# AIoT-MLSys-Lab/Mercury

Measured on AMD Instinct MI355X. Metric: images/sec (whole node) + sampler overhead %, ResNet-18 CIFAR-10 DP 1/2/4/8 GPU, higher is better.
Workload: dtype bf16; 1 GPU; model=resnet18, dataset=cifar10-shape (32x32x3, 10 classes), global_batch=32, per_gpu_batch=32, presample_pool=320, optimizer=adam, parallelism=dp1, sampler=importance (loss + 0.5*EMA), with replacement

## Files before the change

csrc/igemm.h:

```cpp
#pragma once
#include <hip/hip_runtime.h>
#include <stddef.h>

typedef __bf16 bf16;

struct ConvGeom {
  int SH, SW, SC;
  int RP, RQ;
  int R, S, stride, pad;
  int Kc;
  int Ncols;
  int M;
  const bf16* zero;
  int ldb = 0;
  int trb = -1, tsb = 0, tS = 0;
};

constexpr int SUMS_R = 8;

struct EpiParams {
  bf16* out;
  int ldo;
  const float* bias;
  float* stats;
  int stats_ld;
  int group_rows;
  int accumulate;
  float* slab;
  const bf16* bw_out;
  const bf16* bw_y;
  const float* bw_stats;
  const bf16* bw_y2;
  const float* bw_stats2;
  float* bw_sums;
  float bw_inv_count, bw_eps;
  int bw_act;
  int rm_hc = 0, rm_wc = 0, rm_h = 0, rm_w = 0, rm_ph = 0, rm_pw = 0;
};

struct ProParams {
  const float* stats;
  const float* rmean;
  const float* rvar;
  const float* gamma;
  const float* beta;
  bf16* keep;
  int group_rows;
  float inv_count;
  float eps;
  int act;
  int keep_tap;
  const bf16* res = nullptr;
};

size_t igemm_slab_bytes(const ConvGeom& g, int bm, int bn, int splits);
void igemm_launch(const bf16* src, const bf16* wt, const ConvGeom& g, const EpiParams& e, int bm,
                  int bn, int splits, bool trans, hipStream_t st, const ProParams* pro = nullptr);

struct WgradGeom {
  int N, H, W, C;
  int P, Q, K;
  int R, S, stride, pad;
  int Creal;
  const bf16* zero;
  float* slab;
};
void wgrad_launch(const bf16* dy, const bf16* x, const WgradGeom& g, float* dw, int bm, int bn,
                  int splits, hipStream_t st);

int dgrad_s2_launch(const bf16* dy, const bf16* wt, const ConvGeom& g, const EpiParams& e, int bm,
                    int bn, int H, int W, int N, hipStream_t st);

int conv_bwd_pair_s2_launch(const bf16* dy, const bf16* wt, const ConvGeom& g, const EpiParams& e,
                            int bm, int bn, int H, int W, int N, const bf16* x,
                            const WgradGeom& wg, float* dw, int wbm, int wbn, int wsplits,
                            hipStream_t st);

int conv_bwd_pair_launch(const bf16* dy, const bf16* wt, const ConvGeom& g, const EpiParams& e,
                         int bm, int bn, int splits, const bf16* x, const WgradGeom& wg, float* dw,
                         int wbm, int wbn, int wsplits, hipStream_t st);

struct HconvGeom {
  int N, H, W, C;
  int P, Q, K;
  int R, stride, pad;
  int IMG, TR;
  int HT, HWd;
  int HWP, HALF;
  int HS, SR;
  int HPIX;
  int SWA;
  int PGRID;
  int chunks_per_split;
  const bf16* zero;
};

struct HconvPro {
  int mode;
  const float* stats;
  const float* rmean;
  const float* rvar;
  const float* gamma;
  const float* beta;
  int group_imgs;
  float inv_count;
  float eps;
  int act;
  int coef_tab = 0;
};

struct PgemmArgs {
  const bf16* a;
  const bf16* b;
  bf16* out;
  float* stats;
  int M, N, K, ldo, stats_ld, group_rows;
  unsigned a_bytes, b_bytes, out_bytes;
  int H, W, P, Q, stride;
};
struct PgemmPro {
  int mode;
  const float* stats;
  const float* rmean;
  const float* rvar;
  const float* gamma;
  const float* beta;
  float inv_count, eps;
  int act;
  int group_rows;
  int G;
  float* coef;
  const bf16* res;
  bf16* keep;
  unsigned res_bytes, keep_bytes, coef_bytes;
};
int pgemm_launch(const PgemmArgs& g, int bn, int grid, hipStream_t st, const PgemmPro* pro = nullptr);
int pwconv_launch(const PgemmArgs& g, hipStream_t st, const PgemmPro* pro = nullptr);

int hconv_launch(const bf16* src, const bf16* wt, const HconvGeom& g, const EpiParams& e,
                 const HconvPro& pro, int bm, int bn, int splits, hipStream_t st);
const bf16* conv_zero_page();
```

csrc/igemm.hip:

```cpp

#include "conv_epi.h"
#include "wgrad_body.h"

namespace {


__device__ __attribute__((aligned(16))) bf16 g_zero_page[64];

MA_DEV int swz(int row, int chunk) { return chunk ^ (row & 7); }

template <int BM, int BN>
constexpr int nt_occ() { return BM * BN >= 256 * 128 ? 1 : 2; }


template <bool TRANS>
MA_DEV void row_init(const ConvGeom& g, int m, int& off, int& h, int& w) {
  const int pq = g.RP * g.RQ;
  const int mm = m < g.M ? m : 0;
  const int n = udiv24(mm, pq, 1.f / (float)pq), rem = mm - n * pq;
  const int p = udiv24(rem, g.RQ, 1.f / (float)g.RQ), q = rem - p * g.RQ;
  off = m < g.M ? n * g.SH * g.SW : -1;
  h = TRANS ? p + g.pad : p * g.stride - g.pad;
  w = TRANS ? q + g.pad : q * g.stride - g.pad;
}

template <bool TRANS>
MA_DEV int row_at(const ConvGeom& g, int off, int h, int w, int r, int s, int c8) {
  int hh, ww;
  bool ok = off >= 0;
  if (TRANS) {
    const int hp = h - r, wp = w - s;
    if (g.stride == 2) {
      ok = ok && ((hp | wp) & 1) == 0;
      hh = hp >> 1;
      ww = wp >> 1;
    } else {
      hh = hp;
      ww = wp;
    }
  } else {
    hh = h + r;
    ww = w + s;
  }
  ok = ok && (unsigned)hh < (unsigned)g.SH && (unsigned)ww < (unsigned)g.SW;
  const int o = (off + hh * g.SW + ww) * g.SC + c8 * 8;
  return ok ? o : -1;
}

template <bool TRANS>
MA_DEV int row_base(const ConvGeom& g, int off, int h, int w) {
  if (TRANS && g.stride == 2) return (off + (h >> 1) * g.SW + (w >> 1)) * g.SC;
  return (off + h * g.SW + w) * g.SC;
}

template <bool TRANS>
MA_DEV int tap_offset(const ConvGeom& g, int r, int s) {
  if (!TRANS) return (r * g.SW + s) * g.SC;
  if (g.stride == 2) return -((r >> 1) * g.SW + (s >> 1)) * g.SC;
  return -(r * g.SW + s) * g.SC;
}

template <bool TRANS>
MA_DEV bool tap_ok(const ConvGeom& g, int h, int w, int r, int s) {
  if (!TRANS) return (unsigned)(h + r) < (unsigned)g.SH && (unsigned)(w + s) < (unsigned)g.SW;
  const int hp = h - r, wp = w - s;
  if (g.stride == 2)
    return ((hp | wp) & 1) == 0 && (unsigned)(hp >> 1) < (unsigned)g.SH &&
           (unsigned)(wp >> 1) < (unsigned)g.SW;
  return (unsigned)hp < (unsigned)g.SH && (unsigned)wp < (unsigned)g.SW;
}

struct KCursor {
  int tr, ts, tc;
  bool fast;
  MA_DEV void init(const ConvGeom& g, int kt0) {
    const int C8 = g.SC >> 3;
    fast = (C8 & 7) == 0;
    tr = ts = tc = 0;
    if (fast) {
      const int k0c = kt0 * 8;
      const int rs = k0c / C8;
      tc = k0c - rs * C8;
      tr = rs / g.S;
      ts = rs - tr * g.S;
    }
  }
  MA_DEV void decode(const ConvGeom& g, int kt, int lcc, int& r, int& s, int& c8, bool& kval) const {
    const int kc = kt * 8 + lcc;
    kval = kc < g.Kc;
    if (fast) {
      r = tr;
      s = ts;
      c8 = tc + lcc;
    } else {
      const int C8 = g.SC >> 3;
      const int k0 = kt * 8;
      int rs = k0 / C8;
      c8 = k0 - rs * C8 + lcc;
      while (c8 >= C8) {
        c8 -= C8;
        ++rs;
      }
      r = (int)(((float)rs + 0.5f) * (1.f / (float)g.S));
      s = rs - r * g.S;
    }
  }
  MA_DEV void advance(const ConvGeom& g) {
    if (!fast) return;
    tc += 8;
    if (tc == (g.SC >> 3)) {
      tc = 0;
      if (++ts == g.S) {
        ts = 0;
        ++tr;
      }
    }
  }
};

template <int BM, int BN>
MA_DEV void mma_stage(const bf16* a, const bf16* b, f32x4 (&acc)[BM / 32][BN / 32], int lane,
                      int wm, int wn) {
  constexpr int TM = BM / 32, TN = BN / 32;
#pragma unroll
  for (int kk = 0; kk < 2; ++kk) {
    const int chunk = kk * 4 + (lane >> 4);
    bf16x8 fa[TM], fb[TN];
#pragma unroll
    for (int tm = 0; tm < TM; ++tm) {
      const int row = wm * (BM / 2) + tm * 16 + (lane & 15);
      fa[tm] = *(const bf16x8*)(a + row * BK + swz(row, chunk) * 8);
    }
#pragma unroll
    for (int tn = 0; tn < TN; ++tn) {
      const int row = wn * (BN / 2) + tn * 16 + (lane & 15);
      fb[tn] = *(const bf16x8*)(b + row * BK + swz(row, chunk) * 8);
    }
#pragma unroll
    for (int tm = 0; tm < TM; ++tm)
#pragma unroll
      for (int tn = 0; tn < TN; ++tn)
        acc[tm][tn] = __builtin_amdgcn_mfma_f32_16x16x32_bf16(fb[tn], fa[tm], acc[tm][tn], 0, 0, 0);
  }
}

template <int BM, int BN, bool TRANS, bool PRO = false, int PF = 1>
MA_DEV void igemm_nt_body(const bf16* __restrict__ src, const bf16* __restrict__ wt,
                          const ConvGeom& g, const EpiParams& e, int ktiles_per_split, char* smem,
                          int bx, int by, int gx, int gy, const ProParams& pro) {
  constexpr int TM = BM / 32, TN = BN / 32;
  constexpr int AR = BM / 32, BR = BN / 32;
  bf16* sA = (bf16*)smem;

  const int tid = threadIdx.x, lane = tid & 63, w = tid >> 6;
  const int wm = w >> 1, wn = w & 1;
  const int ntn = (g.Ncols + BN - 1) / BN;
  const int mt = bx / ntn, nt = bx - mt * ntn;
  const int m0 = mt * BM, n0 = nt * BN;
  MA_STAMP(0);
  const int ktiles = (g.Kc + 7) / 8;
  const int kt0 = by * ktiles_per_split;
  const int kt1 = min(ktiles, kt0 + ktiles_per_split);
  const int Kelems = g.Kc * 8;
  const int cc = tid & 7;

  int abase[AR], ah[AR], aw[AR];
#pragma unroll
  for (int i = 0; i < AR; ++i) {
    int off;
    row_init<TRANS>(g, m0 + (tid >> 3) + 32 * i, off, ah[i], aw[i]);
    abase[i] = row_base<TRANS>(g, off, ah[i], aw[i]);
    if (off < 0) ah[i] = -(1 << 28);
  }
  int boff[BR];
  const int ldb = g.ldb ? g.ldb : Kelems;
#pragma unroll
  for (int i = 0; i < BR; ++i) {
    const int n = n0 + (tid >> 3) + 32 * i;
    boff[i] = n < g.Ncols ? n * ldb : -1;
  }
  KCursor kc;
  kc.init(g, kt0);
  const bf16* zp = g.zero;

  float4 pst[8];
  int pz = 0;
  int pko[AR];
  u32x4 prs[AR];
  const float* pbase = nullptr;
  if constexpr (PRO) {
    const int grp = m0 / pro.group_rows;
    pbase = pro.stats ? pro.stats + (size_t)grp * 2 * g.SC : nullptr;
  }
  auto load_stage = [&](int kt, u32x4 (&ra)[AR], u32x4 (&rb)[BR]) {
    int r, s, c8;
    bool kval;
    kc.decode(g, kt, cc, r, s, c8, kval);
    kc.advance(g);
    kval = kval && kt < kt1;
    bool keep = false;
    if constexpr (PRO) {
      const int ch = kval ? c8 * 8 : 0;
      const float* m0p = pbase ? pbase + ch : pro.rmean + ch;
      const float* v0p = pbase ? pbase + g.SC + ch : pro.rvar + ch;
      pst[0] = *(const float4*)m0p;
      pst[1] = *(const float4*)(m0p + 4);
      pst[2] = *(const float4*)v0p;
      pst[3] = *(const float4*)(v0p + 4);
      pst[4] = *(const float4*)(pro.gamma + ch);
      pst[5] = *(const float4*)(pro.gamma + ch + 4);
      pst[6] = *(const float4*)(pro.beta + ch);
      pst[7] = *(const float4*)(pro.beta + ch + 4);
      keep = pro.keep != nullptr && nt == 0 && kval && r * g.S + s == pro.keep_tap;
      pz = 0;
    }
    const int toff = tap_offset<TRANS>(g, r, s) + c8 * 8;
    const int bch = g.trb < 0 ? kt * 8 + cc
                              : ((g.trb - 2 * r) * g.tS + (g.tsb - 2 * s)) * (g.SC >> 3) + c8;
#pragma unroll
    for (int i = 0; i < AR; ++i) {
      const bool ok = kval && tap_ok<TRANS>(g, ah[i], aw[i], r, s);
      const int o = abase[i] + toff;
      ra[i] = *(const u32x4*)(ok ? src + o : zp);
      if constexpr (PRO) {
        pz |= (ok ? 0 : 1) << i;
        pko[i] = keep && ok ? o : -1;
        if (pro.res != nullptr) prs[i] = *(const u32x4*)(ok ? pro.res + o : zp);
      }
    }
#pragma unroll
    for (int i = 0; i < BR; ++i) {
      const bool ok = kval && boff[i] >= 0;
      rb[i] = *(const u32x4*)(ok ? wt + boff[i] + bch * 8 : zp);
    }
  };
  auto store_stage = [&](int buf, u32x4 (&ra)[AR], const u32x4 (&rb)[BR]) {
    bf16* a = sA + buf * Smem<BM, BN>::STAGE;
    bf16* b = a + BM * BK;
    if constexpr (PRO) {
      const float mv[8] = {pst[0].x, pst[0].y, pst[0].z, pst[0].w, pst[1].x, pst[1].y, pst[1].z, pst[1].w};
      const float vv[8] = {pst[2].x, pst[2].y, pst[2].z, pst[2].w, pst[3].x, pst[3].y, pst[3].z, pst[3].w};
      const float gv[8] = {pst[4].x, pst[4].y, pst[4].z, pst[4].w, pst[5].x, pst[5].y, pst[5].z, pst[5].w};
      const float bv[8] = {pst[6].x, pst[6].y, pst[6].z, pst[6].w, pst[7].x, pst[7].y, pst[7].z, pst[7].w};
      float sc[8], sh[8];
      float plo, phi;
      act_clamp_bounds(pro.act, plo, phi);
#pragma unroll
      for (int k = 0; k < 8; ++k) {
        float mean = mv[k], var = vv[k];
        if (pbase) {
          mean = mv[k] * pro.inv_count;
          var = fmaxf(vv[k] * pro.inv_count - mean * mean, 0.f);
        }
        sc[k] = gv[k] * rsqrtf(var + pro.eps);
        sh[k] = bv[k] - mean * sc[k];
      }
      const bool hres = pro.res != nullptr;
#pragma unroll
      for (int i = 0; i < AR; ++i) {
        const bf16x8 y = __builtin_bit_cast(bf16x8, ra[i]);
        const bf16x8 rv = __builtin_bit_cast(bf16x8, hres ? prs[i] : u32x4{0u, 0u, 0u, 0u});
        bf16x8 o;
#pragma unroll
        for (int k = 0; k < 8; ++k) {
          o[k] = f2bf(fminf(fmaxf(bf2f(y[k]) * sc[k] + sh[k] + bf2f(rv[k]), plo), phi));
        }
        const u32x4 t = __builtin_bit_cast(u32x4, o);
        ra[i] = ((pz >> i) & 1) ? u32x4{0u, 0u, 0u, 0u} : t;
        if (pko[i] >= 0) *(u32x4*)(pro.keep + pko[i]) = ra[i];
      }
    }
#pragma unroll
    for (int i = 0; i < AR; ++i) {
      const int row = (tid >> 3) + 32 * i;
      *(u32x4*)(a + row * BK + swz(row, cc) * 8) = ra[i];
    }
#pragma unroll
    for (int i = 0; i < BR; ++i) {
      const int row = (tid >> 3) + 32 * i;
      *(u32x4*)(b + row * BK + swz(row, cc) * 8) = rb[i];
    }
  };

  f32x4 acc[TM][TN];
#pragma unroll
  for (int i = 0; i < TM; ++i)
#pragma unroll
    for (int j = 0; j < TN; ++j) acc[i][j] = f32x4{0.f, 0.f, 0.f, 0.f};

  if (kt0 < kt1 && PF == 2) {
    u32x4 ra0[AR], rb0[BR], ra1[AR], rb1[BR];
    load_stage(kt0, ra0, rb0);
    store_stage(0, ra0, rb0);
    load_stage(kt0 + 1, ra1, rb1);
    __syncthreads();
    for (int kt = kt0; kt < kt1; kt += 2) {
      load_stage(kt + 2, ra0, rb0);
      mma_stage<BM, BN>(sA, sA + BM * BK, acc, lane, wm, wn);
      if (kt + 1 >= kt1) break;
      store_stage(1, ra1, rb1);
      __syncthreads();
      load_stage(kt + 3, ra1, rb1);
      const bf16* a1 = sA + Smem<BM, BN>::STAGE;
      mma_stage<BM, BN>(a1, a1 + BM * BK, acc, lane, wm, wn);
      if (kt + 2 >= kt1) break;
      store_stage(0, ra0, rb0);
      __syncthreads();
    }
    __syncthreads();
  } else if (kt0 < kt1) {
    u32x4 ra[AR], rb[BR];
    load_stage(kt0, ra, rb);
    store_stage(0, ra, rb);
    __syncthreads();
    MA_STAMP(1);
#ifdef MERCURY_STAMPS
    unsigned long long lap[4] = {0, 0, 0, 0};
    unsigned long long tl = __builtin_amdgcn_s_memtime();
#endif
    int buf = 0;
    for (int kt = kt0; kt < kt1; ++kt) {
      const bool more = kt + 1 < kt1;
      if (more) load_stage(kt + 1, ra, rb);
      MA_LAP(0, tl);
      const bf16* a = sA + buf * Smem<BM, BN>::STAGE;
      mma_stage<BM, BN>(a, a + BM * BK, acc, lane, wm, wn);
      MA_LAP(1, tl);
      if (more) store_stage(buf ^ 1, ra, rb);
      MA_LAP(2, tl);
      __syncthreads();
      MA_LAP(3, tl);
      buf ^= 1;
    }
#ifdef MERCURY_STAMPS
    if (threadIdx.x == 0) {
      const int b_ = blockIdx.x + blockIdx.y * gridDim.x;
      if (b_ < 8192)
        for (int q = 0; q < 4; ++q) g_stamps[b_][4 + q] = lap[q];
    }
#endif
  }
  MA_STAMP(2);
  finish<BM, BN>(acc, smem, e, g.M, g.Ncols, m0, n0, bx, by, gx, gy);
  MA_STAMP(3);
}


template <int BM, int BN>
constexpr int PAIR_PF() { return BM * BN <= 64 * 128 ? 2 : 1; }

template <int BM, int BN, bool TRANS, int PF = 1>
__global__ __launch_bounds__(NT, (nt_occ<BM, BN>())) void igemm_nt_kernel(const bf16* __restrict__ src,
                                                          const bf16* __restrict__ wt,
                                                          ConvGeom g, EpiParams e,
                                                          int ktiles_per_split) {
  __shared__ __attribute__((aligned(16))) char smem[Smem<BM, BN>::bytes(2)];
  const ProParams none{};
  const int bx = gridDim.y == 1 ? xcd_tile(blockIdx.x, gridDim.x) : blockIdx.x;
  igemm_nt_body<BM, BN, TRANS, false, PF>(src, wt, g, e, ktiles_per_split, smem, bx, blockIdx.y,
                                          gridDim.x, gridDim.y, none);
}

template <int BM, int BN>
__global__ __launch_bounds__(NT, (nt_occ<BM, BN>())) void igemm_pro_kernel(const bf16* __restrict__ src,
                                                           const bf16* __restrict__ wt,
                                                           ConvGeom g, EpiParams e,
                                                           int ktiles_per_split, ProParams pro) {
  __shared__ __attribute__((aligned(16))) char smem[Smem<BM, BN>::bytes(2)];
  const int bx = gridDim.y == 1 ? xcd_tile(blockIdx.x, gridDim.x) : blockIdx.x;
  igemm_nt_body<BM, BN, false, true>(src, wt, g, e, ktiles_per_split, smem, bx,
                                     blockIdx.y, gridDim.x, gridDim.y, pro);
}

template <int BM, int BN, bool TRANS>
void launch_main(const bf16* src, const bf16* wt, const ConvGeom& g, const EpiParams& e, int per,
                 dim3 grid, hipStream_t st) {
  if constexpr (PAIR_PF<BM, BN>() == 2) {
#ifndef MERCURY_FWD_PF1
    if (grid.x * grid.y <= 512) {
      hipLaunchKernelGGL((igemm_nt_kernel<BM, BN, TRANS, 2>), grid, dim3(NT), 0, st, src, wt, g, e,
                         per);
      return;
    }
#endif
  }
  hipLaunchKernelGGL((igemm_nt_kernel<BM, BN, TRANS>), grid, dim3(NT), 0, st, src, wt, g, e, per);
}

inline void ig_grid(const ConvGeom& g, int BM, int BN, int splits, int& gx, int& per, int& gy) {
  const int mtiles = (g.M + BM - 1) / BM, ntiles = (g.Ncols + BN - 1) / BN;
  const int ktiles = (g.Kc + 7) / 8;
  splits = splits < 1 ? 1 : (splits > ktiles ? ktiles : splits);
  per = (ktiles + splits - 1) / splits;
  gy = (ktiles + per - 1) / per;
  gx = mtiles * ntiles;
  if (gx > SEM_INTS) gy = 1, per = ktiles;
}

template <int BM, int BN, bool TRANS>
void launch_cfg(const bf16* src, const bf16* wt, const ConvGeom& g, EpiParams e, int splits,
                hipStream_t st, const ProParams* pro) {
  int gx, per, gy;
  ig_grid(g, BM, BN, splits, gx, per, gy);
  if (gy == 1) e.slab = nullptr;
  if (pro != nullptr && !TRANS) {
    hipLaunchKernelGGL((igemm_pro_kernel<BM, BN>), dim3(gx, gy), dim3(NT), 0, st, src, wt, g, e,
                       per, *pro);
    return;
  }
  launch_main<BM, BN, TRANS>(src, wt, g, e, per, dim3(gx, gy), st);
}

struct IgProb {
  const bf16* src;
  const bf16* wt;
  ConvGeom g;
  EpiParams e;
  int per, gx, gy;
};

template <int BM, int BN, int PF>
__global__ __launch_bounds__(NT, (nt_occ<BM, BN>())) void igemm_dual_kernel(IgProb A, IgProb B) {
  __shared__ __attribute__((aligned(16))) char smem[Smem<BM, BN>::bytes(2)];
  const ProParams none{};
  int b = blockIdx.x;
  const bool first = b < A.gx * A.gy;
  if (!first) b -= A.gx * A.gy;
  const IgProb& p = first ? A : B;
  const int bx0 = b % p.gx, by = b / p.gx;
  const int bx = p.gy == 1 ? xcd_tile(bx0, p.gx) : bx0;
  igemm_nt_body<BM, BN, false, false, PF>(p.src, p.wt, p.g, p.e, p.per, smem, bx, by, p.gx, p.gy,
                                          none);
}

template <int BM, int BN>
void dual_cfg(IgProb A, IgProb B, hipStream_t st) {
  const int grid = A.gx * A.gy + B.gx * B.gy;
  if constexpr (PAIR_PF<BM, BN>() == 2) {
    if (grid <= 512) {
      hipLaunchKernelGGL((igemm_dual_kernel<BM, BN, 2>), dim3(grid), dim3(NT), 0, st, A, B);
      return;
    }
  }
  hipLaunchKernelGGL((igemm_dual_kernel<BM, BN, 1>), dim3(grid), dim3(NT), 0, st, A, B);
}

struct S2Geom {
  ConvGeom g[4];
  int pre[5];
  int hc[4], wc[4];
  int H, W;
};

template <int BM, int BN, int PF>
__global__ __launch_bounds__(NT, (nt_occ<BM, BN>())) void dgrad_s2_kernel(const bf16* __restrict__ dy,
                                                           const bf16* __restrict__ wt,
                                                           S2Geom sg, EpiParams e) {
  __shared__ __attribute__((aligned(16))) char smem[Smem<BM, BN>::bytes(2)];
  const int b = blockIdx.x;
  const int c = (b >= sg.pre[1]) + (b >= sg.pre[2]) + (b >= sg.pre[3]);
  EpiParams ec = e;
  ec.rm_hc = sg.hc[c];
  ec.rm_wc = sg.wc[c];
  ec.rm_h = sg.H;
  ec.rm_w = sg.W;
  ec.rm_ph = c >> 1;
  ec.rm_pw = c & 1;
  const ProParams none{};
  const int bx = b - sg.pre[c];
  igemm_nt_body<BM, BN, false, false, PF>(dy, wt, sg.g[c], ec, 1 << 20, smem, bx, 0,
                                          sg.pre[c + 1] - sg.pre[c], 1, none);
}

template <int BM, int BN>
void s2_cfg(const bf16* dy, const bf16* wt, const S2Geom& sg, const EpiParams& e, hipStream_t st) {
  const int grid = sg.pre[4];
  if (grid == 0) return;
  if constexpr (PAIR_PF<BM, BN>() == 2) {
    if (grid <= 512) {
      hipLaunchKernelGGL((dgrad_s2_kernel<BM, BN, 2>), dim3(grid), dim3(NT), 0, st, dy, wt, sg, e);
      return;
    }
  }
  hipLaunchKernelGGL((dgrad_s2_kernel<BM, BN, 1>), dim3(grid), dim3(NT), 0, st, dy, wt, sg, e);
}

template <int DBM, int DBN, int WBM, int WBN>
__global__ __launch_bounds__(NT, 2) void bwd_pair_kernel(const bf16* __restrict__ dy,
                                                          const bf16* __restrict__ wt, ConvGeom g,
                                                          EpiParams e, int dper, int dgx, int dgy,
                                                          const bf16* __restrict__ x,
                                                          WgradGeom wg, float* __restrict__ dw,
                                                          int wper, int wgx, int wgy) {
  constexpr int DB = Smem<DBM, DBN>::bytes(2), WB = wgb::WgSmem<WBM, WBN>::BYTES;
  __shared__ __attribute__((aligned(16))) char smem[DB > WB ? DB : WB];
  const int nw = wgx * wgy;
  const int b = blockIdx.x;
  if (b < nw) {
    wgb::wgrad_body<WBM, WBN>(dy, x, wg, dw, wper, (bf16*)smem, b % wgx, b / wgx, wgy);
  } else {
    const int d = b - nw;
    const ProParams none{};
    igemm_nt_body<DBM, DBN, true, false, PAIR_PF<DBM, DBN>()>(dy, wt, g, e, dper, smem, d % dgx,
                                                               d / dgx, dgx, dgy, none);
  }
}

template <int DBM, int DBN, int WBM, int WBN>
__global__ __launch_bounds__(NT, 2) void bwd_pair_s2_kernel(const bf16* __restrict__ dy,
                                                             const bf16* __restrict__ wt,
                                                             S2Geom sg, EpiParams e,
                                                             const bf16* __restrict__ x,
                                                             WgradGeom wg, float* __restrict__ dw,
                                                             int wper, int wgx, int wgy) {
  constexpr int DB = Smem<DBM, DBN>::bytes(2), WB = wgb::WgSmem<WBM, WBN>::BYTES;
  __shared__ __attribute__((aligned(16))) char smem[DB > WB ? DB : WB];
  const int nw = wgx * wgy;
  const int b = blockIdx.x;
  if (b < nw) {
    wgb::wgrad_body<WBM, WBN>(dy, x, wg, dw, wper, (bf16*)smem, b % wgx, b / wgx, wgy);
    return;
  }
  const int d = b - nw;
  const int c = (d >= sg.pre[1]) + (d >= sg.pre[2]) + (d >= sg.pre[3]);
  EpiParams ec = e;
  ec.rm_hc = sg.hc[c];
  ec.rm_wc = sg.wc[c];
  ec.rm_h = sg.H;
  ec.rm_w = sg.W;
  ec.rm_ph = c >> 1;
  ec.rm_pw = c & 1;
  const ProParams none{};
  igemm_nt_body<DBM, DBN, false, false, PAIR_PF<DBM, DBN>()>(
      dy, wt, sg.g[c], ec, 1 << 20, smem, d - sg.pre[c], 0, sg.pre[c + 1] - sg.pre[c], 1, none);
}

struct PairProb {
  const bf16* dy;
  const bf16* wt;
  ConvGeom g;
  EpiParams e;
  int dper, dgx, dgy;
  const bf16* x;
  WgradGeom wg;
  float* dw;
  int wper, wgx, wgy;
};
struct S2PairProb {
  const bf16* dy;
  const bf16* wt;
  S2Geom sg;
  EpiParams e;
  const bf16* x;
  WgradGeom wg;
  float* dw;
  int wper, wgx, wgy;
};

template <int DBM, int DBN, int WBM, int WBN>
__global__ __launch_bounds__(NT, 2) void bwd_pair_sc_kernel(PairProb A, S2PairProb B) {
  constexpr int DB = Smem<DBM, DBN>::bytes(2), WB = wgb::WgSmem<WBM, WBN>::BYTES;
  constexpr int SB = Smem<64, 64>::bytes(2), SWB = wgb::WgSmem<64, 64>::BYTES;
  constexpr int M1 = DB > WB ? DB : WB, M2 = SB > SWB ? SB : SWB;
  __shared__ __attribute__((aligned(16))) char smem[M1 > M2 ? M1 : M2];
  const ProParams none{};
  int b = blockIdx.x;
  const int nwA = A.wgx * A.wgy, nA = nwA + A.dgx * A.dgy;
  if (b < nA) {
    if (b < nwA) {
      wgb::wgrad_body<WBM, WBN>(A.dy, A.x, A.wg, A.dw, A.wper, (bf16*)smem, b % A.wgx, b / A.wgx,
                                A.wgy);
    } else {
      const int d = b - nwA;
      igemm_nt_body<DBM, DBN, true, false, PAIR_PF<DBM, DBN>()>(A.dy, A.wt, A.g, A.e, A.dper, smem,
                                                                 d % A.dgx, d / A.dgx, A.dgx,
                                                                 A.dgy, none);
    }
    return;
  }
  b -= nA;
  const int nwB = B.wgx * B.wgy;
  if (b < nwB) {
    wgb::wgrad_body<64, 64>(B.dy, B.x, B.wg, B.dw, B.wper, (bf16*)smem, b % B.wgx, b / B.wgx, B.wgy);
    return;
  }
  const int d = b - nwB;
  const int c = (d >= B.sg.pre[1]) + (d >= B.sg.pre[2]) + (d >= B.sg.pre[3]);
  EpiParams ec = B.e;
  ec.rm_hc = B.sg.hc[c];
  ec.rm_wc = B.sg.wc[c];
  ec.rm_h = B.sg.H;
  ec.rm_w = B.sg.W;
  ec.rm_ph = c >> 1;
  ec.rm_pw = c & 1;
  igemm_nt_body<64, 64, false, false, PAIR_PF<64, 64>()>(B.dy, B.wt, B.sg.g[c], ec, 1 << 20, smem,
                                                         d - B.sg.pre[c], 0,
                                                         B.sg.pre[c + 1] - B.sg.pre[c], 1, none);
}

template <int DBM, int DBN, int WBM, int WBN>
void pair_cfg(const bf16* dy, const bf16* wt, const ConvGeom& g, EpiParams e, int splits,
              const bf16* x, WgradGeom wg, float* dw, int wsplits, hipStream_t st) {
  int dgx, dper, dgy, wgx, wper, wgy;
  ig_grid(g, DBM, DBN, splits, dgx, dper, dgy);
  if (dgy == 1) e.slab = nullptr;
  wgb::wg_grid(wg, WBM, WBN, wsplits, wgx, wper, wgy);
  if (wgx > wgb::WG_SEM_INTS) wg.slab = nullptr;
  hipLaunchKernelGGL((bwd_pair_kernel<DBM, DBN, WBM, WBN>), dim3(dgx * dgy + wgx * wgy), dim3(NT),
                     0, st, dy, wt, g, e, dper, dgx, dgy, x, wg, dw, wper, wgx, wgy);
}

}

int igemm_read_stamps(unsigned long long* host, int n) {
#ifdef MERCURY_STAMPS
  return hipMemcpyFromSymbol(host, HIP_SYMBOL(g_stamps), sizeof(unsigned long long) * 12 * n) ==
         hipSuccess;
#else
  (void)host;
  (void)n;
  return 0;
#endif
}


size_t igemm_slab_bytes(const ConvGeom& g, int bm, int bn, int splits) {
  const size_t mtiles = (g.M + bm - 1) / bm, ntiles = (g.Ncols + bn - 1) / bn;
  return SEM_INTS * 4 + (size_t)splits * mtiles * ntiles * bm * bn * 4;
}

const bf16* conv_zero_page();
static const bf16* zero_page() { return conv_zero_page(); }

const bf16* conv_zero_page() {
  static const bf16* zp = nullptr;
  if (!zp) {
    void* p = nullptr;
    (void)hipGetSymbolAddress(&p, HIP_SYMBOL(g_zero_page));
    zp = (const bf16*)p;
  }
  return zp;
}

void igemm_launch(const bf16* src, const bf16* wt, const ConvGeom& g_in, const EpiParams& e,
                  int bm, int bn, int splits, bool trans, hipStream_t st, const ProParams* pro) {
  ConvGeom g = g_in;
  g.zero = zero_page();
#define MA_CASE(BM_, BN_)                                                           \
  if (bm == BM_ && bn == BN_) {                                                     \
    if (trans) launch_cfg<BM_, BN_, true>(src, wt, g, e, splits, st, nullptr);       \
    else launch_cfg<BM_, BN_, false>(src, wt, g, e, splits, st, pro);                \
    return;                                                                         \
  }
  MA_CASE(128, 128)
  MA_CASE(128, 64)
  MA_CASE(64, 128)
  MA_CASE(64, 64)
  MA_CASE(256, 64)
  MA_CASE(256, 128)
#undef MA_CASE
}

int igemm_dual_launch(const bf16* srcA, const bf16* wtA, const ConvGeom& gA, const EpiParams& eA,
                      int splitsA, const bf16* srcB, const bf16* wtB, const ConvGeom& gB,
                      const EpiParams& eB, int splitsB, int bm, int bn, hipStream_t st) {
  IgProb A{srcA, wtA, gA, eA, 0, 0, 0}, B{srcB, wtB, gB, eB, 0, 0, 0};
  A.g.zero = B.g.zero = zero_page();
  ig_grid(A.g, bm, bn, splitsA, A.gx, A.per, A.gy);
  ig_grid(B.g, bm, bn, splitsB, B.gx, B.per, B.gy);
  if (A.gy == 1) A.e.slab = nullptr;
  if (B.gy == 1) B.e.slab = nullptr;
  if (A.gy > 1 && B.gy > 1 && A.e.slab == B.e.slab) return 0;
#define MA_CASE(BM_, BN_)                 \
  if (bm == BM_ && bn == BN_) {           \
    dual_cfg<BM_, BN_>(A, B, st);         \
    return 1;                             \
  }
  MA_CASE(64, 128)
  MA_CASE(128, 128)
  MA_CASE(128, 64)
  MA_CASE(64, 64)
#undef MA_CASE
  return 0;
}

static bool s2_geom(const ConvGeom& gt, int bm, int bn, int H, int W, int N, S2Geom& sg) {
  if (gt.stride != 2 || (gt.SC & 63) || gt.R != gt.S) return false;
  if (!((gt.R == 3 && gt.pad == 1) || (gt.R == 1 && gt.pad == 0))) return false;
  sg = S2Geom{};
  sg.H = H;
  sg.W = W;
  sg.pre[0] = 0;
  for (int c = 0; c < 4; ++c) {
    const int ph = c >> 1, pw = c & 1;
    int rv = 0, trb = -1;
    for (int r = gt.R - 1; r >= 0; --r)
      if (((ph + gt.pad - r) & 1) == 0) {
        if (trb < 0) trb = r;
        ++rv;
      }
    int sv = 0, tsb = -1;
    for (int s = gt.S - 1; s >= 0; --s)
      if (((pw + gt.pad - s) & 1) == 0) {
        if (tsb < 0) tsb = s;
        ++sv;
      }
    if ((rv && ph + gt.pad - trb != 0) || (sv && pw + gt.pad - tsb != 0)) return false;
    const int hc = (H - ph + 1) / 2, wc = (W - pw + 1) / 2;
    ConvGeom g{};
    g.SH = gt.SH;
    g.SW = gt.SW;
    g.SC = gt.SC;
    g.RP = hc;
    g.RQ = wc;
    g.R = rv > 0 ? rv : 1;
    g.S = sv > 0 ? sv : 1;
    g.stride = 1;
    g.pad = 0;
    g.Kc = (rv * sv) * (gt.SC >> 3);
    g.Ncols = gt.Ncols;
    g.M = N * hc * wc;
    g.zero = zero_page();
    g.ldb = gt.R * gt.S * gt.SC;
    g.trb = trb < 0 ? 0 : trb;
    g.tsb = tsb < 0 ? 0 : tsb;
    g.tS = gt.S;
    sg.g[c] = g;
    sg.hc[c] = hc;
    sg.wc[c] = wc;
    sg.pre[c + 1] = sg.pre[c] + ((g.M + bm - 1) / bm) * ((g.Ncols + bn - 1) / bn);
  }
  return true;
}

int dgrad_s2_launch(const bf16* dy, const bf16* wt, const ConvGeom& gt, const EpiParams& e_in,
                    int bm, int bn, int H, int W, int N, hipStream_t st) {
  S2Geom sg;
  if (!s2_geom(gt, bm, bn, H, W, N, sg)) return 0;
  EpiParams e = e_in;
  e.slab = nullptr;
#define MA_CASE(BM_, BN_)                    \
  if (bm == BM_ && bn == BN_) {              \
    s2_cfg<BM_, BN_>(dy, wt, sg, e, st);     \
    return 1;                                \
  }
  MA_CASE(128, 128)
  MA_CASE(128, 64)
  MA_CASE(64, 128)
  MA_CASE(64, 64)
  MA_CASE(256, 64)
#undef MA_CASE
  return 0;
}

int conv_bwd_pair_s2_launch(const bf16* dy, const bf16* wt, const ConvGeom& gt,
                            const EpiParams& e_in, int bm, int bn, int H, int W, int N,
                            const bf16* x, const WgradGeom& wg_in, float* dw, int wbm, int wbn,
                            int wsplits, hipStream_t st) {
  S2Geom sg;
  if (!s2_geom(gt, bm, bn, H, W, N, sg)) return 0;
  EpiParams e = e_in;
  e.slab = nullptr;
  WgradGeom wg = wg_in;
  wg.zero = zero_page();
#define MA_W(DBM_, DBN_, WBM_, WBN_)                                                        \
  if (bm == DBM_ && bn == DBN_ && wbm == WBM_ && wbn == WBN_) {                            \
    int wgx, wper, wgy;                                                                    \
    wgb::wg_grid(wg, WBM_, WBN_, wsplits, wgx, wper, wgy);                                 \
    if (wgx > wgb::WG_SEM_INTS) wg.slab = nullptr;                                         \
    hipLaunchKernelGGL((bwd_pair_s2_kernel<DBM_, DBN_, WBM_, WBN_>),                        \
                       dim3(sg.pre[4] + wgx * wgy), dim3(NT), 0, st, dy, wt, sg, e, x, wg, dw, \
                       wper, wgx, wgy);                                                    \
    return 1;                                                                              \
  }
  MA_W(64, 64, 64, 64)
  MA_W(64, 64, 128, 128)
  MA_W(64, 64, 64, 128)
  MA_W(64, 64, 128, 64)
#undef MA_W
  return 0;
}

int conv_bwd_pair_sc_launch(const bf16* dyA, const bf16* wtA, const ConvGeom& gA_in,
                            const EpiParams& eA_in, int bm, int bn, int splits, const bf16* xA,
                            const WgradGeom& wgA_in, float* dwA, int wbm, int wbn,
                            int wsplits, const bf16* dyB, const bf16* wtB, const ConvGeom& gtB,
                            const EpiParams& eB_in, int HB, int WB, int NB, const bf16* xB,
                            const WgradGeom& wgB_in, float* dwB, int wsplitsB,
                            hipStream_t st) {
  PairProb A;
  A.dy = dyA;
  A.wt = wtA;
  A.g = gA_in;
  A.g.zero = zero_page();
  A.e = eA_in;
  A.x = xA;
  A.wg = wgA_in;
  A.wg.zero = A.g.zero;
  A.dw = dwA;
  ig_grid(A.g, bm, bn, splits, A.dgx, A.dper, A.dgy);
  if (A.dgy == 1) A.e.slab = nullptr;
  wgb::wg_grid(A.wg, wbm, wbn, wsplits, A.wgx, A.wper, A.wgy);
  if (A.wgx > wgb::WG_SEM_INTS) A.wg.slab = nullptr;
  S2PairProb B;
  if (!s2_geom(gtB, 64, 64, HB, WB, NB, B.sg)) return 0;
  B.dy = dyB;
  B.wt = wtB;
  B.e = eB_in;
  B.e.slab = nullptr;
  B.x = xB;
  B.wg = wgB_in;
  B.wg.zero = A.g.zero;
  B.dw = dwB;
  wgb::wg_grid(B.wg, 64, 64, wsplitsB, B.wgx, B.wper, B.wgy);
  if (B.wgx > wgb::WG_SEM_INTS) B.wg.slab = nullptr;
  if (A.wg.slab != nullptr && A.wg.slab == B.wg.slab) return 0;
  const int grid = A.wgx * A.wgy + A.dgx * A.dgy + B.wgx * B.wgy + B.sg.pre[4];
#define MA_SC(DBM_, DBN_, WBM_, WBN_)                                                       \
  if (bm == DBM_ && bn == DBN_ && wbm == WBM_ && wbn == WBN_) {                             \
    hipLaunchKernelGGL((bwd_pair_sc_kernel<DBM_, DBN_, WBM_, WBN_>), dim3(grid), dim3(NT), 0, st, \
                       A, B);                                                                \
    return 1;                                                                                \
  }
  MA_SC(64, 64, 64, 64)
  MA_SC(64, 64, 128, 128)
#undef MA_SC
  return 0;
}

int conv_bwd_pair_launch(const bf16* dy, const bf16* wt, const ConvGeom& g_in, const EpiParams& e,
                         int bm, int bn, int splits, const bf16* x, const WgradGeom& wg_in,
                         float* dw, int wbm, int wbn, int wsplits, hipStream_t st) {
  ConvGeom g = g_in;
  g.zero = zero_page();
  WgradGeom wg = wg_in;
  wg.zero = g.zero;
#define MA_W(DBM_, DBN_, WBM_, WBN_)                                                   \
  if (wbm == WBM_ && wbn == WBN_) {                                                   \
    pair_cfg<DBM_, DBN_, WBM_, WBN_>(dy, wt, g, e, splits, x, wg, dw, wsplits, st);   \
    return 1;                                                                         \
  }
#define MA_D(DBM_, DBN_)                                                               \
  if (bm == DBM_ && bn == DBN_) {                                                     \
    MA_W(DBM_, DBN_, 128, 128)                                                        \
    MA_W(DBM_, DBN_, 128, 64)                                                         \
    MA_W(DBM_, DBN_, 64, 128)                                                         \
    MA_W(DBM_, DBN_, 64, 64)                                                          \
  }
  MA_D(128, 128)
  MA_D(128, 64)
  MA_D(64, 128)
  MA_D(64, 64)
  MA_D(256, 64)
#undef MA_D
#undef MA_W
  return 0;
}
```

csrc/wgrad_body.h:

```cpp
#pragma once
#include "common.h"
#include "igemm.h"

namespace wgb {
constexpr int WG_NT = 256;
constexpr int WG_BKP = 64;
constexpr int WG_SEM_INTS = 1024;

typedef short short4_t __attribute__((ext_vector_type(4)));

MA_DEV bf16x4 tr_read(const bf16* p) {
  short4_t v = __builtin_amdgcn_ds_read_tr16_b64_v4i16(
      (__attribute__((address_space(3))) short4_t*)(p));
  return __builtin_bit_cast(bf16x4, v);
}

template <int BM, int BN>
struct WgSmem {
  static constexpr int STAGE = WG_BKP * ((BM + 16) + (BN + 16));
  static constexpr int BYTES = 2 * STAGE * 2;
};

template <int BM, int BN, int PF = (BM * BN <= 64 * 128 ? 2 : 1)>
MA_DEV void wgrad_body(const bf16* __restrict__ dy, const bf16* __restrict__ x, const WgradGeom& g,
                       float* __restrict__ dw, int ptiles_per_split, bf16* smem, int bx, int by,
                       int gy) {
  constexpr int NT = WG_NT, BKP = WG_BKP;
  constexpr int LDA = BM + 16, LDB = BN + 16;
  constexpr int STAGE = WgSmem<BM, BN>::STAGE;
  constexpr int TM = BM / 32, TN = BN / 32;
  constexpr int ACH = BM / 8, BCH = BN / 8;
  constexpr int AR = BKP * ACH / NT, BR = BKP * BCH / NT;

  const int tid = threadIdx.x, lane = tid & 63, w = tid >> 6;
  const int wm = w >> 1, wn = w & 1;
  const int C8 = g.C >> 3;
  const int Kc = g.R * g.S * C8;
  const int ncols = Kc * 8;
  const int ntn = (ncols + BN - 1) / BN;
  const int mt = bx / ntn, nt = bx - mt * ntn;
  const int m0 = mt * BM, n0 = nt * BN;
  const int npix = g.N * g.P * g.Q;
  const int ptiles = (npix + BKP - 1) / BKP;
  const int pt0 = by * ptiles_per_split;
  const int pt1 = min(ptiles, pt0 + ptiles_per_split);

  const int bcc = tid % BCH;
  const int jc = n0 / 8 + bcc;
  int xr = 0, xs = 0, xc8 = 0;
  const bool jval = jc < Kc;
  if (jval) {
    const int rs = jc / C8;
    xc8 = jc - rs * C8;
    xr = rs / g.S;
    xs = rs - xr * g.S;
  }
  const int acc_ = tid % ACH;

  const auto rdy = __builtin_amdgcn_make_buffer_rsrc((void*)dy, 0, npix * g.K * 2, 0x00020000);
  const auto rx = __builtin_amdgcn_make_buffer_rsrc((void*)x, 0, g.N * g.H * g.W * g.C * 2,
                                                    0x00020000);
  constexpr unsigned BAD = 0x80000000u;
  const int k = m0 + acc_ * 8;
  int pixA = pt0 * BKP + tid / ACH;
  const bool pw = g.R == 1 && g.S == 1 && g.stride == 1 && g.pad == 0;
  const int aq = BKP % g.Q, ap = BKP / g.Q;
  int pixB = pt0 * BKP + tid / BCH;
  int bn_[BR], bp_[BR], bq_[BR];
#pragma unroll
  for (int i = 0; i < BR; ++i) {
    const int pix = pixB + i * (NT / BCH);
    const int pq = g.P * g.Q;
    bn_[i] = pix / pq;
    const int rem = pix - bn_[i] * pq;
    bp_[i] = rem / g.Q;
    bq_[i] = rem - bp_[i] * g.Q;
  }
  auto load_stage = [&](int pt, u32x4 (&ra)[AR], u32x4 (&rb)[BR]) {
    const bool live = pt < pt1;
#pragma unroll
    for (int i = 0; i < AR; ++i) {
      const int pix = pixA + i * (NT / ACH);
      const bool ok = live && pix < npix && k < g.K;
      ra[i] = __builtin_bit_cast(u32x4, __builtin_amdgcn_raw_buffer_load_b128(
                                            rdy, ok ? (unsigned)(pix * g.K + k) * 2u : BAD, 0, 0));
    }
    pixA += BKP;
#pragma unroll
    for (int i = 0; i < BR; ++i) {
      unsigned off;
      bool ok;
      if (pw) {
        const int pix = pixB + i * (NT / BCH);
        ok = live && jval && pix < npix;
        off = (unsigned)(pix * g.C + xc8 * 8) * 2u;
      } else {
        const int h = bp_[i] * g.stride - g.pad + xr, ww = bq_[i] * g.stride - g.pad + xs;
        ok = live && jval && bn_[i] < g.N && (unsigned)h < (unsigned)g.H &&
             (unsigned)ww < (unsigned)g.W;
        off = (unsigned)(((bn_[i] * g.H + h) * g.W + ww) * g.C + xc8 * 8) * 2u;
        int q = bq_[i] + aq, p = bp_[i] + ap, n = bn_[i];
        if (q >= g.Q) {
          q -= g.Q;
          ++p;
        }
        while (p >= g.P) {
          p -= g.P;
          ++n;
        }
        bn_[i] = n;
        bp_[i] = p;
        bq_[i] = q;
      }
      rb[i] = __builtin_bit_cast(u32x4,
                                 __builtin_amdgcn_raw_buffer_load_b128(rx, ok ? off : BAD, 0, 0));
    }
    pixB += BKP;
  };
  auto store_stage = [&](int buf, const u32x4 (&ra)[AR], const u32x4 (&rb)[BR]) {
    bf16* a = smem + buf * STAGE;
    bf16* b = a + BKP * LDA;
#pragma unroll
    for (int i = 0; i < AR; ++i) {
      const int row = tid / ACH + i * (NT / ACH);
      *(u32x4*)(a + row * LDA + acc_ * 8) = ra[i];
    }
#pragma unroll
    for (int i = 0; i < BR; ++i) {
      const int row = tid / BCH + i * (NT / BCH);
      *(u32x4*)(b + row * LDB + bcc * 8) = rb[i];
    }
  };

  f32x4 acc[TM][TN];
#pragma unroll
  for (int i = 0; i < TM; ++i)
#pragma unroll
    for (int j = 0; j < TN; ++j) acc[i][j] = f32x4{0.f, 0.f, 0.f, 0.f};

  const int g4 = lane >> 4, li = lane & 15;
  const int tq = li >> 2, tp = li & 3;
  auto mma = [&](int buf) {
    const bf16* a = smem + buf * STAGE;
    const bf16* b = a + BKP * LDA;
#pragma unroll
    for (int kk = 0; kk < 2; ++kk) {
      bf16x8 fa[TM], fb[TN];
#pragma unroll
      for (int h = 0; h < 2; ++h) {
        const int row = kk * 32 + 16 * h + 4 * g4 + tq;
#pragma unroll
        for (int tm = 0; tm < TM; ++tm) {
          const bf16x4 v = tr_read(a + row * LDA + wm * (BM / 2) + tm * 16 + 4 * tp);
#pragma unroll
          for (int e = 0; e < 4; ++e) fa[tm][4 * h + e] = v[e];
        }
#pragma unroll
        for (int tn = 0; tn < TN; ++tn) {
          const bf16x4 v = tr_read(b + row * LDB + wn * (BN / 2) + tn * 16 + 4 * tp);
#pragma unroll
          for (int e = 0; e < 4; ++e) fb[tn][4 * h + e] = v[e];
        }
      }
#pragma unroll
      for (int tm = 0; tm < TM; ++tm)
#pragma unroll
        for (int tn = 0; tn < TN; ++tn)
          acc[tm][tn] = __builtin_amdgcn_mfma_f32_16x16x32_bf16(fa[tm], fb[tn], acc[tm][tn], 0, 0, 0);
    }
  };
  if (pt0 < pt1 && PF == 1) {
    u32x4 ra[AR], rb[BR];
    load_stage(pt0, ra, rb);
    store_stage(0, ra, rb);
    __syncthreads();
    int buf = 0;
    for (int pt = pt0; pt < pt1; ++pt) {
      const bool more = pt + 1 < pt1;
      if (more) load_stage(pt + 1, ra, rb);
      mma(buf);
      if (more) store_stage(buf ^ 1, ra, rb);
      __syncthreads();
      buf ^= 1;
    }
  } else if (pt0 < pt1) {
    u32x4 ra0[AR], rb0[BR], ra1[AR], rb1[BR];
    load_stage(pt0, ra0, rb0);
    store_stage(0, ra0, rb0);
    load_stage(pt0 + 1, ra1, rb1);
    __syncthreads();
    for (int pt = pt0; pt < pt1; pt += 2) {
      load_stage(pt + 2, ra0, rb0);
      mma(0);
      if (pt + 1 >= pt1) break;
      store_stage(1, ra1, rb1);
      __syncthreads();
      load_stage(pt + 3, ra1, rb1);
      mma(1);
      if (pt + 2 >= pt1) break;
      store_stage(0, ra0, rb0);
      __syncthreads();
    }
  }

  bool atomic = gy > 1;
  if (atomic && g.slab != nullptr) {
    atomic = false;
    const int ntiles = (g.K + BM - 1) / BM * ntn;
    int* sem = (int*)g.slab;
    const auto rs = __builtin_amdgcn_make_buffer_rsrc((void*)(g.slab + WG_SEM_INTS), 0,
                                                      0x7fffffff, 0x00020000);
    constexpr int tile_bytes = TM * TN * NT * 16;
    const int mine = (by * ntiles + bx) * tile_bytes + tid * 16;
#pragma unroll
    for (int tm = 0; tm < TM; ++tm)
#pragma unroll
      for (int tn = 0; tn < TN; ++tn)
        __builtin_amdgcn_raw_buffer_store_b128(__builtin_bit_cast(u32x4, acc[tm][tn]), rs,
                                               mine + (tm * TN + tn) * NT * 16, 0, 16 );
    asm volatile("s_waitcnt vmcnt(0)" ::: "memory");
    int* flag = (int*)smem;
    __syncthreads();
    if (tid == 0) {
      const int old = __hip_atomic_fetch_add(&sem[bx], 1, __ATOMIC_RELAXED,
                                             __HIP_MEMORY_SCOPE_AGENT);
      const int last = old == gy - 1;
      if (last) __hip_atomic_store(&sem[bx], 0, __ATOMIC_RELAXED, __HIP_MEMORY_SCOPE_AGENT);
      flag[0] = last;
    }
    __syncthreads();
    if (!flag[0]) return;
    __builtin_amdgcn_fence(__ATOMIC_ACQUIRE, "wavefront");
    for (int sp = 0; sp < gy; ++sp) {
      if (sp == by) continue;
      const int base = (sp * ntiles + bx) * tile_bytes + tid * 16;
#pragma unroll
      for (int tm = 0; tm < TM; ++tm)
#pragma unroll
        for (int tn = 0; tn < TN; ++tn)
          acc[tm][tn] += __builtin_bit_cast(
              f32x4, __builtin_amdgcn_raw_buffer_load_b128(rs, base + (tm * TN + tn) * NT * 16, 0,
                                                           16 ));
    }
  }
  const int RSCr = g.R * g.S * g.Creal;
#pragma unroll
  for (int tn = 0; tn < TN; ++tn) {
    const int col = n0 + wn * (BN / 2) + tn * 16 + li;
    if (col >= ncols) continue;
    const int rs = col / g.C, c = col - rs * g.C;
    if (c >= g.Creal) continue;
#pragma unroll
    for (int tm = 0; tm < TM; ++tm) {
#pragma unroll
      for (int j = 0; j < 4; ++j) {
        const int k = m0 + wm * (BM / 2) + tm * 16 + g4 * 4 + j;
        if (k >= g.K) continue;
        float* dst = dw + (size_t)k * RSCr + rs * g.Creal + c;
        if (atomic) atomicAdd(dst, acc[tm][tn][j]);
        else *dst = acc[tm][tn][j];
      }
    }
  }
}

inline void wg_grid(const WgradGeom& g, int bm, int bn, int splits, int& gx, int& per, int& gy) {
  const int ncols = g.R * g.S * g.C;
  const int mtiles = (g.K + bm - 1) / bm, ntiles = (ncols + bn - 1) / bn;
  const int ptiles = (g.N * g.P * g.Q + WG_BKP - 1) / WG_BKP;
  splits = splits < 1 ? 1 : (splits > ptiles ? ptiles : splits);
  per = (ptiles + splits - 1) / splits;
  gy = (ptiles + per - 1) / per;
  gx = mtiles * ntiles;
}

inline size_t wg_slab_bytes(int gx, int gy, int bm, int bn) {
  return (size_t)WG_SEM_INTS * 4 + (size_t)gx * gy * bm * bn * 4;
}
}
```

Measured before the change: 25280 trained images/s.

## Use buffer loads with OOB masking in igemm and incremental offsets in wgrad

Switches the implicit-GEMM A/B/residual loads from flat pointer loads with a zero-page fallback to raw buffer loads, where an out-of-bounds offset returns zero. Per-row tap validity is precomputed as H/W bitmasks, so the per-tap bounds check becomes a single mask test. In wgrad, the per-stage n/p/q recomputation with a while loop is replaced by incremental byte-offset updates using conditional wraparound. A host-side range check now limits tensors to under 4 GB because offsets are 32-bit. The intent is fewer address and compare instructions in the inner load loops and less VGPR use.

Result: faster. 25790 trained images/s (median of 6 runs) (+2.0%).

```diff
diff --git a/csrc/igemm.h b/csrc/igemm.h
--- a/csrc/igemm.h
+++ b/csrc/igemm.h
@@ -14,7 +14,11 @@
   const bf16* zero;
   int ldb = 0;
   int trb = -1, tsb = 0, tS = 0;
+  unsigned a_bytes = 0, b_bytes = 0;
 };
+
+constexpr long long IGEMM_RANGE_LIM = 0xFFFFFF00LL;
+void igemm_ranges(ConvGeom& g, long long images, const char* who);
 
 constexpr int SUMS_R = 8;
 
diff --git a/csrc/igemm.hip b/csrc/igemm.hip
--- a/csrc/igemm.hip
+++ b/csrc/igemm.hip
@@ -1,3 +1,6 @@
+
+#include <stdexcept>
+#include <string>
 
 #include "conv_epi.h"
 #include "wgrad_body.h"
@@ -61,13 +64,30 @@
 }
 
 template <bool TRANS>
-MA_DEV bool tap_ok(const ConvGeom& g, int h, int w, int r, int s) {
-  if (!TRANS) return (unsigned)(h + r) < (unsigned)g.SH && (unsigned)(w + s) < (unsigned)g.SW;
-  const int hp = h - r, wp = w - s;
-  if (g.stride == 2)
-    return ((hp | wp) & 1) == 0 && (unsigned)(hp >> 1) < (unsigned)g.SH &&
-           (unsigned)(wp >> 1) < (unsigned)g.SW;
-  return (unsigned)hp < (unsigned)g.SH && (unsigned)wp < (unsigned)g.SW;
+MA_DEV unsigned axis_mask(int x, int E, int T, int stride) {
+  int lo, hi;
+  unsigned par = ~0u;
+  if (!TRANS) {
+    lo = -x;
+    hi = E - x;
+  } else if (stride == 2) {
+    lo = x - 2 * E + 1;
+    hi = x + 1;
+    par = (x & 1) ? 0xAAu : 0x55u;
+  } else {
+    lo = x - E + 1;
+    hi = x + 1;
+  }
+  lo = min(max(lo, 0), 8);
+  hi = min(max(hi, 0), T);
+  return ((1u << hi) - 1u) & ~((1u << lo) - 1u) & par;
+}
+
+constexpr unsigned IG_OOB = 0xFFFFFF00u;
+constexpr int IG_RSRC_FLAGS = 0x00020000;
+
+MA_DEV u32x4 ig_load16(__amdgpu_buffer_rsrc_t rs, unsigned byte_off) {
+  return __builtin_bit_cast(u32x4, __builtin_amdgcn_raw_buffer_load_b128(rs, byte_off, 0, 0));
 }
 
 struct KCursor {
@@ -164,34 +184,43 @@
   const int Kelems = g.Kc * 8;
   const int cc = tid & 7;
 
-  int abase[AR], ah[AR], aw[AR];
+  const auto rsa = __builtin_amdgcn_make_buffer_rsrc((void*)src, 0, g.a_bytes, IG_RSRC_FLAGS);
+  const auto rsb = __builtin_amdgcn_make_buffer_rsrc((void*)wt, 0, g.b_bytes, IG_RSRC_FLAGS);
+
+  unsigned abase[AR], amask[AR];
 #pragma unroll
   for (int i = 0; i < AR; ++i) {
-    int off;
-    row_init<TRANS>(g, m0 + (tid >> 3) + 32 * i, off, ah[i], aw[i]);
-    abase[i] = row_base<TRANS>(g, off, ah[i], aw[i]);
-    if (off < 0) ah[i] = -(1 << 28);
-  }
-  int boff[BR];
+    int off, h, w;
+    row_init<TRANS>(g, m0 + (tid >> 3) + 32 * i, off, h, w);
+    abase[i] = (unsigned)row_base<TRANS>(g, off, h, w) * 2u;
+    const unsigned hm = axis_mask<TRANS>(h, g.SH, g.R, g.stride);
+    const unsigned wm = axis_mask<TRANS>(w, g.SW, g.S, g.stride);
+    amask[i] = off >= 0 ? hm | (wm << 8) : 0u;
+  }
+  unsigned boff[BR];
+  bool bval[BR];
   const int ldb = g.ldb ? g.ldb : Kelems;
 #pragma unroll
   for (int i = 0; i < BR; ++i) {
     const int n = n0 + (tid >> 3) + 32 * i;
-    boff[i] = n < g.Ncols ? n * ldb : -1;
+    bval[i] = n < g.Ncols;
+    boff[i] = (unsigned)n * (unsigned)ldb * 2u;
   }
   KCursor kc;
   kc.init(g, kt0);
-  const bf16* zp = g.zero;
 
   float4 pst[8];
   int pz = 0;
-  int pko[AR];
+  unsigned pko[AR];
   u32x4 prs[AR];
   const float* pbase = nullptr;
   if constexpr (PRO) {
     const int grp = m0 / pro.group_rows;
     pbase = pro.stats ? pro.stats + (size_t)grp * 2 * g.SC : nullptr;
   }
+  const auto rsr = __builtin_amdgcn_make_buffer_rsrc(
+      (void*)(PRO ? pro.res : nullptr), 0, PRO && pro.res != nullptr ? g.a_bytes : 0u,
+      IG_RSRC_FLAGS);
   auto load_stage = [&](int kt, u32x4 (&ra)[AR], u32x4 (&rb)[BR]) {
     int r, s, c8;
     bool kval;
@@ -214,24 +243,26 @@
       keep = pro.keep != nullptr && nt == 0 && kval && r * g.S + s == pro.keep_tap;
       pz = 0;
     }
-    const int toff = tap_offset<TRANS>(g, r, s) + c8 * 8;
+    const unsigned toff = (unsigned)(tap_offset<TRANS>(g, r, s) + c8 * 8) * 2u;
+    const unsigned tbits = kval ? (1u << r) | (0x100u << s) : 0x80000000u;
     const int bch = g.trb < 0 ? kt * 8 + cc
                               : ((g.trb - 2 * r) * g.tS + (g.tsb - 2 * s)) * (g.SC >> 3) + c8;
+    const unsigned bcol = (unsigned)bch * 16u;
 #pragma unroll
     for (int i = 0; i < AR; ++i) {
-      const bool ok = kval && tap_ok<TRANS>(g, ah[i], aw[i], r, s);
-      const int o = abase[i] + toff;
-      ra[i] = *(const u32x4*)(ok ? src + o : zp);
+      const bool ok = (amask[i] & tbits) == tbits;
+      const unsigned o = ok ? abase[i] + toff : IG_OOB;
+      ra[i] = ig_load16(rsa, o);
       if constexpr (PRO) {
         pz |= (ok ? 0 : 1) << i;
-        pko[i] = keep && ok ? o : -1;
-        if (pro.res != nullptr) prs[i] = *(const u32x4*)(ok ? pro.res + o : zp);
+        pko[i] = keep ? o : IG_OOB;
+        if (pro.res != nullptr) prs[i] = ig_load16(rsr, o);
       }
     }
 #pragma unroll
     for (int i = 0; i < BR; ++i) {
-      const bool ok = kval && boff[i] >= 0;
-      rb[i] = *(const u32x4*)(ok ? wt + boff[i] + bch * 8 : zp);
+      const bool ok = kval && bval[i];
+      rb[i] = ig_load16(rsb, ok ? boff[i] + bcol : IG_OOB);
     }
   };
   auto store_stage = [&](int buf, u32x4 (&ra)[AR], const u32x4 (&rb)[BR]) {
@@ -267,7 +298,7 @@
         }
         const u32x4 t = __builtin_bit_cast(u32x4, o);
         ra[i] = ((pz >> i) & 1) ? u32x4{0u, 0u, 0u, 0u} : t;
-        if (pko[i] >= 0) *(u32x4*)(pro.keep + pko[i]) = ra[i];
+        if (pko[i] != IG_OOB) *(u32x4*)((char*)pro.keep + pko[i]) = ra[i];
       }
     }
 #pragma unroll
@@ -642,10 +673,27 @@
   return zp;
 }
 
+void igemm_ranges(ConvGeom& g, long long images, const char* who) {
+  const long long a = images * g.SH * g.SW * g.SC * 2;
+  const long long ldb = g.ldb ? (long long)g.ldb : (long long)g.Kc * 8;
+  const long long b = (long long)g.Ncols * ldb * 2;
+  if (images < 0 || a < 0 || b < 0 || a >= IGEMM_RANGE_LIM || b >= IGEMM_RANGE_LIM)
+    throw std::invalid_argument(std::string(who) +
+                                ": tensors must be < 4 GB (32-bit buffer offsets)");
+  g.a_bytes = (unsigned)a;
+  g.b_bytes = (unsigned)b;
+}
+
+static long long geom_images(const ConvGeom& g) {
+  const long long pq = (long long)g.RP * g.RQ;
+  return pq > 0 ? g.M / pq : 0;
+}
+
 void igemm_launch(const bf16* src, const bf16* wt, const ConvGeom& g_in, const EpiParams& e,
                   int bm, int bn, int splits, bool trans, hipStream_t st, const ProParams* pro) {
   ConvGeom g = g_in;
   g.zero = zero_page();
+  igemm_ranges(g, geom_images(g), "igemm");
 #define MA_CASE(BM_, BN_)                                                           \
   if (bm == BM_ && bn == BN_) {                                                     \
     if (trans) launch_cfg<BM_, BN_, true>(src, wt, g, e, splits, st, nullptr);       \
@@ -666,6 +714,8 @@
                       const EpiParams& eB, int splitsB, int bm, int bn, hipStream_t st) {
   IgProb A{srcA, wtA, gA, eA, 0, 0, 0}, B{srcB, wtB, gB, eB, 0, 0, 0};
   A.g.zero = B.g.zero = zero_page();
+  igemm_ranges(A.g, geom_images(A.g), "igemm_dual");
+  igemm_ranges(B.g, geom_images(B.g), "igemm_dual");
   ig_grid(A.g, bm, bn, splitsA, A.gx, A.per, A.gy);
   ig_grid(B.g, bm, bn, splitsB, B.gx, B.per, B.gy);
   if (A.gy == 1) A.e.slab = nullptr;
@@ -725,6 +775,7 @@
     g.trb = trb < 0 ? 0 : trb;
     g.tsb = tsb < 0 ? 0 : tsb;
     g.tS = gt.S;
+    igemm_ranges(g, N, "dgrad_s2");
     sg.g[c] = g;
     sg.hc[c] = hc;
     sg.wc[c] = wc;
@@ -793,6 +844,7 @@
   A.wt = wtA;
   A.g = gA_in;
   A.g.zero = zero_page();
+  igemm_ranges(A.g, geom_images(A.g), "conv_bwd_pair_sc");
   A.e = eA_in;
   A.x = xA;
   A.wg = wgA_in;
@@ -833,6 +885,7 @@
                          float* dw, int wbm, int wbn, int wsplits, hipStream_t st) {
   ConvGeom g = g_in;
   g.zero = zero_page();
+  igemm_ranges(g, geom_images(g), "conv_bwd_pair");
   WgradGeom wg = wg_in;
   wg.zero = g.zero;
 #define MA_W(DBM_, DBN_, WBM_, WBN_)                                                   \
diff --git a/csrc/wgrad_body.h b/csrc/wgrad_body.h
--- a/csrc/wgrad_body.h
+++ b/csrc/wgrad_body.h
@@ -64,17 +64,26 @@
   const int k = m0 + acc_ * 8;
   int pixA = pt0 * BKP + tid / ACH;
   const bool pw = g.R == 1 && g.S == 1 && g.stride == 1 && g.pad == 0;
-  const int aq = BKP % g.Q, ap = BKP / g.Q;
+  const int pqB = g.P * g.Q;
+  const int an = BKP / pqB, arem = BKP - an * pqB;
+  const int ap = arem / g.Q, aq = arem - ap * g.Q;
+  const int xrow = g.W * g.C * 2, xpix = g.C * 2;
+  const int dstage = an * g.H * xrow + ap * g.stride * xrow + aq * g.stride * xpix;
+  const int dq = g.stride * xrow - g.Q * g.stride * xpix;
+  const int dp = g.H * xrow - g.P * g.stride * xrow;
+  const int wlim = g.Q * g.stride - g.pad + xs, hlim = g.P * g.stride - g.pad + xr;
   int pixB = pt0 * BKP + tid / BCH;
-  int bn_[BR], bp_[BR], bq_[BR];
+  int bh_[BR], bw_[BR];
+  unsigned bo_[BR];
 #pragma unroll
   for (int i = 0; i < BR; ++i) {
     const int pix = pixB + i * (NT / BCH);
-    const int pq = g.P * g.Q;
-    bn_[i] = pix / pq;
-    const int rem = pix - bn_[i] * pq;
-    bp_[i] = rem / g.Q;
-    bq_[i] = rem - bp_[i] * g.Q;
+    const int n = pix / pqB;
+    const int rem = pix - n * pqB;
+    const int p = rem / g.Q, q = rem - p * g.Q;
+    bh_[i] = p * g.stride - g.pad + xr;
+    bw_[i] = q * g.stride - g.pad + xs;
+    bo_[i] = (unsigned)(((n * g.H + bh_[i]) * g.W + bw_[i]) * g.C + xc8 * 8) * 2u;
   }
   auto load_stage = [&](int pt, u32x4 (&ra)[AR], u32x4 (&rb)[BR]) {
     const bool live = pt < pt1;
@@ -95,22 +104,24 @@
         ok = live && jval && pix < npix;
         off = (unsigned)(pix * g.C + xc8 * 8) * 2u;
       } else {
-        const int h = bp_[i] * g.stride - g.pad + xr, ww = bq_[i] * g.stride - g.pad + xs;
-        ok = live && jval && bn_[i] < g.N && (unsigned)h < (unsigned)g.H &&
+        const int pix = pixB + i * (NT / BCH);
+        int h = bh_[i], ww = bw_[i];
+        ok = live && jval && pix < npix && (unsigned)h < (unsigned)g.H &&
              (unsigned)ww < (unsigned)g.W;
-        off = (unsigned)(((bn_[i] * g.H + h) * g.W + ww) * g.C + xc8 * 8) * 2u;
-        int q = bq_[i] + aq, p = bp_[i] + ap, n = bn_[i];
-        if (q >= g.Q) {
-          q -= g.Q;
-          ++p;
-        }
-        while (p >= g.P) {
-          p -= g.P;
-          ++n;
-        }
-        bn_[i] = n;
-        bp_[i] = p;
-        bq_[i] = q;
+        off = bo_[i];
+        unsigned o = off + (unsigned)dstage;
+        h += ap * g.stride;
+        ww += aq * g.stride;
+        const bool cq = ww >= wlim;
+        ww -= cq ? g.Q * g.stride : 0;
+        h += cq ? g.stride : 0;
+        o += cq ? (unsigned)dq : 0u;
+        const bool cp = h >= hlim;
+        h -= cp ? g.P * g.stride : 0;
+        o += cp ? (unsigned)dp : 0u;
+        bh_[i] = h;
+        bw_[i] = ww;
+        bo_[i] = o;
       }
       rb[i] = __builtin_bit_cast(u32x4,
                                  __builtin_amdgcn_raw_buffer_load_b128(rx, ok ? off : BAD, 0, 0));
```
